# Jiawei-Yang/Denoising-ViT

Measured on AMD Instinct MI355X. Metric: stage-1 images denoised/sec (DINOv2-B/14, 518px, 1k Adam steps), higher is better.
Workload: dtype bf16

## Files before the change

### denoising-vit_amd/csrc/dvt_common.h

```cpp
#pragma once
#include <hip/hip_runtime.h>
#include <stdint.h>

#include "../../include/dvt_hip.h"

#define DVT_CHECK_LAUNCH()                         \
  do {                                             \
    hipError_t e__ = hipGetLastError();            \
    if (e__ != hipSuccess) return (int)e__;        \
  } while (0)

static inline int dvt_cdiv(long long a, long long b) { return (int)((a + b - 1) / b); }

__device__ __forceinline__ float wave_sum(float v) {
#pragma unroll
  for (int o = 32; o > 0; o >>= 1) v += __shfl_xor(v, o, 64);
  return v;
}

__device__ __forceinline__ double wave_sum_f64(double v) {
#pragma unroll
  for (int o = 32; o > 0; o >>= 1) v += __shfl_xor(v, o, 64);
  return v;
}
// ... 131 lines not shown
          t[dvt_frag_off32(k + 0, n, N)] = v.x;
          t[dvt_frag_off32(k + 1, n, N)] = v.y;
          t[dvt_frag_off32(k + 2, n, N)] = v.z;
          t[dvt_frag_off32(k + 3, n, N)] = v.w;
        }
        continue;
      }
      const uint32_t lo = dvt_pack_bf16x2(v.x, v.y), hi = dvt_pack_bf16x2(v.z, v.w);
      *reinterpret_cast<uint2*>(sh + L.direct[i] + dvt_frag_off(n, k, K)) = make_uint2(lo, hi);
      if (L.transp[i] >= 0) {
        uint16_t* t = sh + L.transp[i];
        t[dvt_frag_off(k + 0, n, N)] = (uint16_t)(lo & 0xffffu);
        t[dvt_frag_off(k + 1, n, N)] = (uint16_t)(lo >> 16);
        t[dvt_frag_off(k + 2, n, N)] = (uint16_t)(hi & 0xffffu);
        t[dvt_frag_off(k + 3, n, N)] = (uint16_t)(hi >> 16);
      }
    }
  }
}
#endif
bool dvt_fit_fused_ok(const DvtFitConfig* c);
bool dvt_fit_fused_shapes_ok(const DvtFitConfig* c);
int dvt_fit_rows_k(const DvtFitConfig* c, const DvtShadowLayout* L, int k, const DvtFusedFit* fits, bool phase2,
                   hipStream_t s);
int dvt_fit_backward_k(const DvtFitConfig* c, int k, const DvtFusedFit* fits, bool phase2, hipStream_t s);

extern unsigned g_dvt_prof_mask;
long dvt_prof_begin(int probe, hipStream_t s, unsigned long long* gen);
void dvt_prof_end(int probe, long idx, unsigned long long gen, hipStream_t s, double work);
struct DvtProbeScope {
  int probe;
  hipStream_t s;
  double work;
  long idx;
  unsigned long long gen;
  DvtProbeScope(int p, hipStream_t st, double w) : probe(p), s(st), work(w), idx(-1), gen(0) {
    if ((g_dvt_prof_mask >> p) & 1u) idx = dvt_prof_begin(probe, s, &gen);
  }
  ~DvtProbeScope() {
    if (idx >= 0) dvt_prof_end(probe, idx, gen, s, work);
  }
};
int dvt_vit_tune(int gemm_variant);
int dvt_grid_tune(int lds_level_max);
int dvt_adam_tune(int zero_all);
int dvt_s2_tune(int mask);

// ... 33 lines not shown
```

### denoising-vit_amd/csrc/dvt_fit.hip

```cpp
#include <math.h>

#include "dvt_common.h"
#include "dvt_grid_dev.h"

extern int g_fit_sorted_grid;
#ifdef DVT_LAB
int g_fit_skip_mask = 0;
#endif
int g_fit_lazy_adam = 1;
int g_fit_shadow_in_adam = 1;
int g_fit_lazy_merge = 1;
int g_fit_lazy_exact = 0;
int g_fit_lazy_refresh = 32;

int g_adam_pingpong = 1;

namespace {

inline int64_t up256(int64_t x) { return (x + 255) / 256 * 256; }

struct Work {
  float *enc, *h1, *F, *raw, *dF, *dh1, *denc, *rows, *r1, *r2, *Hres, *dH, *dr2, *dr1;
  int32_t* g_offs;
  uint16_t* g_perm;
  void* shadow;
  void* T;
  uint32_t* gs_keys;
  uint16_t* gs_pay;
// ... 157 lines not shown
  return dvt_linear_fwd(h1, params + c->off_w2, params + c->off_b2, out, n, c->feat_dim,
                        c->hidden, 0, s);
}

namespace {

#define DVT_TRY(x)         \
  do {                     \
    int rc__ = (x);        \
    if (rc__) return rc__; \
  } while (0)

int check_bufs(const DvtFitConfig* c, const DvtFitBuffers* b, int step_begin, int step_end) {
  int rc = check_cfg(c);
  if (rc) return rc;
  if (!b || !b->feat || !b->xy || !b->idx || !b->params || !b->adam_m || !b->adam_v ||
      !b->grads || !b->touched || !b->workspace || !b->h_lr)
    return DVT_E_BADARG;
  if (step_begin < 0 || step_end > c->num_iters || step_begin > step_end) return DVT_E_BADARG;
  return 0;
}

int fit_step(const DvtFitConfig* c, int k, const DvtFitBuffers* const* bs, const Work* ws, int step,
             int gs_local, uint32_t lazy_e0, const DvtAdamLazy* lazy_next, int lazy_target, bool fused, hipStream_t s) {
  const int B = c->batch, C = c->feat_dim, H = c->hidden, R = c->res_hidden;
  const int E = c->grid.n_levels * c->grid.n_features;
  const bool phase2 = step > c->switch_step;
  const bool use_res = phase2 && c->enable_residual;
  constexpr int KM = DVT_FIT_BATCH_MAX;
  const float* xy[KM];
  const int32_t* ridx[KM];
  const float* feat[KM];
  float *P[KM], *Gd[KM], *M[KM], *V[KM];
  uint32_t* touched[KM];
  for (int f = 0; f < k; ++f) {
    xy[f] = bs[f]->xy;
    ridx[f] = bs[f]->idx + (size_t)step * B;
    feat[f] = bs[f]->feat;
    P[f] = bs[f]->params;
    Gd[f] = bs[f]->grads;
    M[f] = bs[f]->adam_m;
    V[f] = bs[f]->adam_v;
    touched[f] = bs[f]->touched;
  }
  auto at = [&](float* const* base, int64_t off, float** out) {
    for (int f = 0; f < k; ++f) out[f] = base[f] + off;
  };
// ... 20 lines not shown
    return o;
  };
  DvtLinearOp ops[4 * KM];
  int n_ops;
  auto launch = [&]() { return dvt_linear_group(ops, n_ops, s, c->mlp_bf16); };
  DvtShadowLayout shl{};
  void* shadow[KM] = {nullptr, nullptr, nullptr, nullptr};
  DvtFusedFit ff[KM];
  if (fused) {
    DVT_TRY(dvt_shadow_layout(c, &shl));
    for (int f = 0; f < k; ++f) {
      const Work& w = ws[f];
      shadow[f] = w.shadow;
      const size_t gso = (size_t)gs_local * c->grid.n_levels * 4 * B;
      const bool gs = w.gs_keys != nullptr && gs_local >= 0;
      ff[f] = DvtFusedFit{xy[f], ridx[f], feat[f], P[f], w.shadow, w.T, w.F, w.Hres, w.dF, w.denc, w.rows, Gd[f],
                          w.g_offs + (size_t)step * (c->lattice + 1), w.g_perm + (size_t)step * B, touched[f],
                          gs ? w.gs_keys + gso : nullptr, gs ? w.gs_pay + gso : nullptr, gs ? w.gs_w + gso : nullptr,
                          lazy_e0};
    }
#ifdef DVT_LAB
    if (!(g_fit_skip_mask & 1))
#endif
    DVT_TRY(dvt_fit_rows_k(c, &shl, k, ff, use_res, s));
  } else {
  {
    float* gridp[KM];
    at(P, c->off_grid, gridp);
    DVT_TRY(dvt_fit_prep_k(&c->grid, k, xy, ridx, gridp, enc, feat, raw, B, C, s));
  }
  n_ops = 0;
  for (int f = 0; f < k; ++f) {
    const Work& w = ws[f];
    ops[n_ops++] = fwd_op(f, w.enc, c->off_w1, c->off_b1, w.h1, H, E, 1);
    if (use_res) ops[n_ops++] = fwd_op(f, w.raw, c->off_wh1, c->off_bh1, w.r1, R, C, 1);
  }
  DVT_TRY(launch());
  n_ops = 0;
  for (int f = 0; f < k; ++f) {
    const Work& w = ws[f];
    ops[n_ops++] = fwd_op(f, w.h1, c->off_w2, c->off_b2, w.F, C, H, 0);
    if (use_res) ops[n_ops++] = fwd_op(f, w.r1, c->off_wh2, c->off_bh2, w.r2, R, R, 1);
  }
  DVT_TRY(launch());
  if (use_res) {
    n_ops = 0;
    for (int f = 0; f < k; ++f) ops[n_ops++] = fwd_op(f, ws[f].r2, c->off_wh3, c->off_bh3, ws[f].Hres, C, R, 0);
// ... 144 lines not shown
  return dvt_fit_run_batched(c, 1, &b, step_begin, step_end, stream);
}

extern "C" int dvt_fit_run_batched(const DvtFitConfig* c, int k, const DvtFitBuffers* const* bufs,
                                   int step_begin, int step_end, void* stream) {
  if (k <= 0 || k > DVT_FIT_BATCH_MAX || !bufs) return DVT_E_BADARG;
  Work w[DVT_FIT_BATCH_MAX];
  for (int j = 0; j < k; ++j) {
    int rc = check_bufs(c, bufs[j], step_begin, step_end);
    if (rc) return rc;
    for (int i = 0; i < j; ++i)
      if (bufs[i]->params == bufs[j]->params || bufs[i]->workspace == bufs[j]->workspace)
        return DVT_E_BADARG;
    carve(c, bufs[j]->workspace, &w[j]);
    if (w[j].g_offs != nullptr && step_begin < c->switch_step + 1) {
      const int last = step_end < c->switch_step + 1 ? step_end : c->switch_step + 1;
      rc = dvt_build_row_lists(bufs[j]->idx + (size_t)step_begin * c->batch, last - step_begin, c->batch,
                               c->lattice, w[j].g_offs + (size_t)step_begin * (c->lattice + 1),
                               w[j].g_perm + (size_t)step_begin * c->batch, (hipStream_t)stream);
      if (rc) return rc;
    }
  }
  const bool fused = dvt_fit_fused_ok(c) && w[0].shadow != nullptr && w[0].g_offs != nullptr;
  if (fused && step_end > step_begin) {
    DvtShadowLayout L;
    int rc = dvt_shadow_layout(c, &L);
    if (rc) return rc;
    const float* pp[DVT_FIT_BATCH_MAX];
    void* ss[DVT_FIT_BATCH_MAX];
    for (int j = 0; j < k; ++j) {
      pp[j] = bufs[j]->params;
      ss[j] = w[j].shadow;
    }
    rc = dvt_shadow_build_k(&L, k, pp, ss, 0, c->arena_floats, (hipStream_t)stream);
    if (rc) return rc;
  }
  const bool sorted_lists = g_fit_fused_enable_lists(c) && w[0].g_offs != nullptr && w[0].gs_keys != nullptr && g_fit_sorted_grid;
  uint32_t lazy_e0 = 0xffffffffu;
  int lazy_l0 = 0;
  DvtAdamLazy lz{};
  const int n_call = step_end - step_begin;
  const bool lazy = sorted_lists && g_fit_lazy_adam && w[0].lazy_done != nullptr && n_call >= 1 && n_call <= 65535 &&
                    lazy_range(c, &lazy_e0, &lazy_l0);
  if (!lazy) lazy_e0 = 0xffffffffu;
  if (lazy) {
    lz.e0 = lazy_e0;
// ... 47 lines not shown
          uc[j] = w[j].gs_ucount;
        }
        int rc = dvt_grid_sort_k(&c->grid, k, xy, ridx, c->batch, steps, keys, pay, ww, (hipStream_t)stream,
                                 lazy ? uk : nullptr, lazy ? uc : nullptr);
        if (rc) return rc;
      }
    }
    if (lazy && step > step_begin && (step - step_begin) % g_fit_lazy_refresh == 0) {
      int rc = dvt_adam_lazy_k(&lz, k, true, step - step_begin, nullptr, nullptr, (hipStream_t)stream);
      if (rc) return rc;
    } else if (lazy && step > step_begin && !merged_catchup) {
      const uint32_t* uk[DVT_FIT_BATCH_MAX];
      const int32_t* uc[DVT_FIT_BATCH_MAX];
      for (int j = 0; j < k; ++j) {
        uk[j] = w[j].gs_ukeys + (size_t)gs_local * c->grid.n_levels * 4 * c->batch;
        uc[j] = w[j].gs_ucount + (size_t)gs_local * c->grid.n_levels;
      }
      int rc = dvt_adam_lazy_k(&lz, k, false, step - step_begin, uk, uc, (hipStream_t)stream);
      if (rc) return rc;
    }
    const int rel_next = step + 1 - step_begin;
    merged_catchup = lazy && g_fit_lazy_merge && step + 1 < step_end && gs_local + 1 < GS_CHUNK &&
                     rel_next % g_fit_lazy_refresh != 0;
    int rc = fit_step(c, k, bufs, w, step, gs_local, lazy_e0, merged_catchup ? &lz : nullptr, rel_next, fused, (hipStream_t)stream);
    if (rc) return rc;
  }
  if (lazy) {
    int rc = dvt_adam_lazy_k(&lz, k, true, n_call, nullptr, nullptr, (hipStream_t)stream);
    if (rc) return rc;
  }
  return 0;
}
```

### denoising-vit_amd/csrc/dvt_fit_fused.hip

```cpp
#include "dvt_common.h"
#include "dvt_grid_dev.h"
#include "dvt_loss_row.h"

typedef short bf16x8 __attribute__((ext_vector_type(8)));
typedef float f32x4 __attribute__((ext_vector_type(4)));

int g_fit_rows32 = 1;
int g_fit_xcd_affinity = 1;
int g_fit_small_wg = 0;

namespace {

constexpr int FR0 = 16;
constexpr int FW8 = 8;
constexpr int FE = 128;

template <bool F32>
struct Op {
  static constexpr int ES = F32 ? 4 : 2;
  static constexpr int KS = F32 ? 16 : 32;
};
typedef unsigned u32x4f __attribute__((ext_vector_type(4)));

template <bool F32>
__host__ __device__ constexpr int apitch(int K) { return K * Op<F32>::ES + 16; }

struct FusedArgs {
  DvtGridTable T;
  DvtShadowLayout S;
  DvtTLayout TL;
  int n, lattice;
// ... 16 lines not shown
      const int sg = brow >> 4, g = (brow >> 2) & 3;
      float4 v;
      v.x = *reinterpret_cast<const float*>(src);
      v.y = *reinterpret_cast<const float*>(src + apitch<F32>(NC));
      v.z = *reinterpret_cast<const float*>(src + 2 * apitch<F32>(NC));
      v.w = *reinterpret_cast<const float*>(src + 3 * apitch<F32>(NC));
      const long long off = ((long long)(col >> 4) * (B >> 4) + sg) * 256 + (((g << 4) + (col & 15)) << 2);
      *reinterpret_cast<float4*>(static_cast<float*>(dstTv) + off) = v;
    } else {
      const int kstep = brow >> 5, g = (brow >> 3) & 3;
      uint32_t w[4];
#pragma unroll
      for (int j = 0; j < 4; ++j) {
        const uint32_t lo = *reinterpret_cast<const uint16_t*>(src + (2 * j) * apitch<F32>(NC));
        const uint32_t hi = *reinterpret_cast<const uint16_t*>(src + (2 * j + 1) * apitch<F32>(NC));
        w[j] = lo | (hi << 16);
      }
      const long long off = ((long long)(col >> 4) * (B >> 5) + kstep) * 512 + (((g << 4) + (col & 15)) << 3);
      *reinterpret_cast<uint4*>(static_cast<uint16_t*>(dstTv) + off) = make_uint4(w[0], w[1], w[2], w[3]);
    }
  }
}

template <int K, int N, bool RELU, bool MASK, int RB, int FW, bool F32>
__device__ __forceinline__ void mlp_layer(const char* actA, const void* __restrict__ Wv,
                                          const float* __restrict__ bias, char* act_out,
                                          float* __restrict__ gout, const char* mask, int wave, int lane) {
  constexpr int KS = Op<F32>::KS, ES = Op<F32>::ES;
  constexpr int NTILES = N / 16, NT = (NTILES + FW - 1) / FW, S = K / KS;
  constexpr int INFL = FW == 8 ? 24 : 16;
  constexpr int PD0 = INFL / NT > 16 ? 16 : (INFL / NT < 1 ? 1 : INFL / NT);
  constexpr int PD = PD0 < S ? PD0 : S;
  static_assert(K % KS == 0 && N % 16 == 0, "layer shape");
  const int lc = lane & 15, g = lane >> 4;
  f32x4 acc[RB][NT];
  const char* wp[NT];
#pragma unroll
  for (int i = 0; i < NT; ++i) {
#pragma unroll
    for (int rb = 0; rb < RB; ++rb) acc[rb][i] = (f32x4){0.f, 0.f, 0.f, 0.f};
    const int t = wave + FW * i;
    const int tt = (NTILES % FW == 0 || t < NTILES) ? t : 0;
    wp[i] = static_cast<const char*>(Wv) + (size_t)tt * S * 1024 + lane * 16;
  }
  u32x4f b[PD][NT];
#pragma unroll
  for (int p = 0; p < PD; ++p)
#pragma unroll
    for (int i = 0; i < NT; ++i) b[p][i] = *reinterpret_cast<const u32x4f*>(wp[i] + 1024 * p);
  __builtin_amdgcn_sched_barrier(0);
  const char* ap = actA + lc * apitch<F32>(K) + g * 16;
#pragma unroll
  for (int s = 0; s < S; ++s) {
    u32x4f av[RB];
#pragma unroll
    for (int rb = 0; rb < RB; ++rb) av[rb] = *reinterpret_cast<const u32x4f*>(ap + rb * 16 * apitch<F32>(K) + s * 64);
    if constexpr (F32) {
#pragma unroll
      for (int j = 0; j < 4; ++j)
#pragma unroll
        for (int i = 0; i < NT; ++i)
#pragma unroll
          for (int rb = 0; rb < RB; ++rb)
            acc[rb][i] = __builtin_amdgcn_mfma_f32_16x16x4f32(__uint_as_float(av[rb][j]), __uint_as_float(b[s % PD][i][j]),
                                                              acc[rb][i], 0, 0, 0);
    } else {
#pragma unroll
      for (int i = 0; i < NT; ++i)
#pragma unroll
        for (int rb = 0; rb < RB; ++rb)
          acc[rb][i] = __builtin_amdgcn_mfma_f32_16x16x32_bf16(__builtin_bit_cast(bf16x8, av[rb]),
                                                               __builtin_bit_cast(bf16x8, b[s % PD][i]), acc[rb][i], 0, 0, 0);
    }
    if (s + PD < S) {
#pragma unroll
      for (int i = 0; i < NT; ++i) b[s % PD][i] = *reinterpret_cast<const u32x4f*>(wp[i] + 1024 * (s + PD));
    }
    __builtin_amdgcn_sched_barrier(0);
  }
#pragma unroll
  for (int i = 0; i < NT; ++i) {
    const int t = wave + FW * i;
    if (NTILES % FW != 0 && t >= NTILES) continue;
    const int n = t * 16 + lc;
    const float bv = bias != nullptr ? bias[n] : 0.f;
#pragma unroll
    for (int rb = 0; rb < RB; ++rb)
#pragma unroll
      for (int r = 0; r < 4; ++r) {
        const int row = rb * 16 + 4 * g + r;
        float v = acc[rb][i][r] + bv;
        if (RELU) v = fmaxf(v, 0.f);
        if (MASK) {
          if constexpr (F32) {
            v = *reinterpret_cast<const float*>(mask + row * apitch<F32>(N) + n * ES) > 0.f ? v : 0.f;
          } else {
            const uint16_t m = *reinterpret_cast<const uint16_t*>(mask + row * apitch<F32>(N) + n * ES);
            v = (m != 0 && !(m & 0x8000u)) ? v : 0.f;
          }
        }
        if (act_out != nullptr) {
          if constexpr (F32) *reinterpret_cast<float*>(act_out + row * apitch<F32>(N) + n * ES) = v;
          else *reinterpret_cast<uint16_t*>(act_out + row * apitch<F32>(N) + n * ES) = bf16_of(v);
        }
        if (gout != nullptr) gout[(size_t)row * N + n] = v;
      }
  }
}

template <int C, bool PH2, int FR, bool F32 = false>
struct FusedLds {
  static constexpr int H = C / 2, R = C / 4;
  static constexpr int O_ENC = 0;
  static constexpr int O_H1 = O_ENC + FR * apitch<F32>(FE);
  static constexpr int O_DF = O_H1 + FR * apitch<F32>(H);
  static constexpr int O_RAW = O_DF + FR * apitch<F32>(C);
  static constexpr int O_R1 = O_RAW + FR * apitch<F32>(C);
  static constexpr int O_R2 = O_R1 + FR * apitch<F32>(R);
  static constexpr int TOTAL = PH2 ? O_R2 + FR * apitch<F32>(R) : O_RAW;
};
template <int C>
constexpr bool fused_f32_fits() { return FusedLds<C, true, 16, true>::TOTAL <= 160 * 1024; }

template <int C, bool PH2, int FR, int FW, bool F32 = false>
__global__ __launch_bounds__(64 * FW) void fit_rows_kernel(FusedArgs a) {
  using L = FusedLds<C, PH2, FR, F32>;
  constexpr int RB = FR / 16;
  constexpr int ES = Op<F32>::ES;
  static_assert(FR == 16 || FR == 32, "rows per workgroup");
  static_assert(FW == 8 || (FW == 4 && FR == 16), "waves per workgroup");
  static_assert(!F32 || (FR == 16 && FW == 8), "fp32 operands: 16 rows, 8 waves");
  static_assert(L::TOTAL <= 160 * 1024, "LDS images of the row kernel");
  constexpr int H = C / 2, R = C / 4, E = FE, cq = C / 4;
  __shared__ __attribute__((aligned(16))) char smem[L::TOTAL];
  int fit_, rb_;
  if (a.xcd_group > 0) {
    const int lin = (int)blockIdx.x + (int)blockIdx.y * (int)gridDim.x, xcd = lin & 7, j = lin >> 3;
    fit_ = xcd / a.xcd_group;
    rb_ = j * a.xcd_group + xcd % a.xcd_group;
  } else {
    fit_ = (int)blockIdx.y;
    rb_ = (int)blockIdx.x;
  }
  const DvtFusedFit& f = a.f[fit_];
  const int tid = threadIdx.x, lane = tid & 63;
  const int wave = __builtin_amdgcn_readfirstlane(tid >> 6);
  const int row0 = rb_ * FR;
// ... 9 lines not shown
    for (int rr = lane / 32; rr < FR / FW; rr += 2) {
      if (j < LPR) {
        const int ri = f.ridx[row0 + wave + FW * rr];
        warm[4] ^= __float_as_uint(f.feat[(size_t)ri * C + j * 32]) ^
                   __float_as_uint(P[a.off_G + (size_t)(ri % a.lattice) * C + j * 32]);
      }
    }
  }
  {
    const int per_xcd = a.xcd_group > 0 ? (int)gridDim.x / a.xcd_group : ((int)gridDim.x + 7) / 8;
    const int nslot = per_xcd >= 16 ? 16 : per_xcd;
    const int slot = (a.xcd_group > 0 ? rb_ / a.xcd_group : (rb_ >> 3)) % nslot;
    const long long lines = ((PH2 ? a.S.total : a.S.direct[2]) * ES + 127) / 128;
    const long long per = (lines + nslot - 1) / nslot;
    const long long l0 = slot * per, l1 = l0 + per < lines ? l0 + per : lines;
    const uint32_t* w32 = reinterpret_cast<const uint32_t*>(sh);
#pragma unroll
    for (int j = 0; j < 4 * RB * (8 / FW); ++j) {
      const long long li = l0 + tid + (long long)j * 64 * FW;
      if (li < l1) warm[j & 3] ^= w32[li * 32];
    }
  }

  if (tid < FR * 16) {
    const int r = tid >> 4, l = tid & 15;
    const float2 p = reinterpret_cast<const float2*>(f.xy)[f.ridx[row0 + r]];
    uint32_t idx[4];
    float w[4];
    corners2d(a.T, l, p.x, p.y, idx, w);
    const float4* __restrict__ grid = reinterpret_cast<const float4*>(P + a.off_grid);
    float4 lo = make_float4(0.f, 0.f, 0.f, 0.f), hi = lo;
#pragma unroll
    for (int c = 0; c < 4; ++c) {
      const float4 u = grid[(size_t)idx[c] * 2], v = grid[(size_t)idx[c] * 2 + 1];
      lo.x = fmaf(w[c], u.x, lo.x);
      lo.y = fmaf(w[c], u.y, lo.y);
      lo.z = fmaf(w[c], u.z, lo.z);
      lo.w = fmaf(w[c], u.w, lo.w);
      hi.x = fmaf(w[c], v.x, hi.x);
      hi.y = fmaf(w[c], v.y, hi.y);
      hi.z = fmaf(w[c], v.z, hi.z);
      hi.w = fmaf(w[c], v.w, hi.w);
    }
    if constexpr (F32) {
      *reinterpret_cast<float4*>(smem + L::O_ENC + r * apitch<F32>(E) + l * 32) = lo;
      *reinterpret_cast<float4*>(smem + L::O_ENC + r * apitch<F32>(E) + l * 32 + 16) = hi;
    } else {
      *reinterpret_cast<uint4*>(smem + L::O_ENC + r * apitch<F32>(E) + l * 16) =
          make_uint4(dvt_pack_bf16x2(lo.x, lo.y), dvt_pack_bf16x2(lo.z, lo.w), dvt_pack_bf16x2(hi.x, hi.y),
                     dvt_pack_bf16x2(hi.z, hi.w));
    }
  }
  if (PH2) {
    for (int i = tid; i < FR * cq; i += 64 * FW) {
      const int r = i / cq, q = i - r * cq;
      const float4 v = feat4[(size_t)f.ridx[row0 + r] * cq + q];
      if constexpr (F32)
        *reinterpret_cast<float4*>(smem + L::O_RAW + r * apitch<F32>(C) + q * 16) = v;
      else
        *reinterpret_cast<uint2*>(smem + L::O_RAW + r * apitch<F32>(C) + q * 8) =
            make_uint2(dvt_pack_bf16x2(v.x, v.y), dvt_pack_bf16x2(v.z, v.w));
    }
  }
  __syncthreads();

  const int B = a.n;
  char* __restrict__ T = static_cast<char*>(f.T);
#define SH(off) (sh + (size_t)(off) * ES)
#define TT(idx) (T + (size_t)a.TL.off[idx] * ES)
  mlp_layer<E, H, true, false, RB, FW, F32>(smem + L::O_ENC, SH(a.S.direct[0]), P + a.off_b1, smem + L::O_H1, nullptr,
                               nullptr, wave, lane);
  if (PH2)
    mlp_layer<C, R, true, false, RB, FW, F32>(smem + L::O_RAW, SH(a.S.direct[2]), P + a.off_bh1, smem + L::O_R1, nullptr,
                                 nullptr, wave, lane);
  __syncthreads();
  mlp_layer<H, C, false, false, RB, FW, F32>(smem + L::O_H1, SH(a.S.direct[1]), P + a.off_b2, nullptr,
                                f.F + (size_t)row0 * C, nullptr, wave, lane);
  store_T<H, FR, FW, F32>(smem + L::O_H1, TT(DVT_T_H1), B, row0, tid);
  store_T<E, FR, FW, F32>(smem + L::O_ENC, TT(DVT_T_ENC), B, row0, tid);
  if (PH2) {
    mlp_layer<R, R, true, false, RB, FW, F32>(smem + L::O_R1, SH(a.S.direct[3]), P + a.off_bh2, smem + L::O_R2, nullptr,
                                 nullptr, wave, lane);
    store_T<C, FR, FW, F32>(smem + L::O_RAW, TT(DVT_T_RAW), B, row0, tid);
    store_T<R, FR, FW, F32>(smem + L::O_R1, TT(DVT_T_R1), B, row0, tid);
    __syncthreads();
    mlp_layer<R, C, false, false, RB, FW, F32>(smem + L::O_R2, SH(a.S.direct[4]), P + a.off_bh3, nullptr,
                                  f.Hres + (size_t)row0 * C, nullptr, wave, lane);
    store_T<R, FR, FW, F32>(smem + L::O_R2, TT(DVT_T_R2), B, row0, tid);
  }
  __syncthreads();

  static_assert(C <= 1024, "row warm-up above assumes <= 32 lines per row");
  {
    constexpr int NR = FR / FW;
    constexpr int NB = (C <= 768 && !(FW == 4 && PH2)) ? 2 : 1;
    DvtLossRowRegs<PH2> lr[NB];
#pragma unroll
    for (int r0 = 0; r0 < NR; r0 += NB) {
#pragma unroll
    for (int rr = r0; rr < r0 + NB; ++rr) {
      const int gr = row0 + wave + FW * rr;
      const int ri = f.ridx[gr];
      dvt_loss_row_load<PH2>(lr[rr - r0], reinterpret_cast<const float4*>(f.F) + (size_t)gr * cq,
                             reinterpret_cast<const float4*>(P + a.off_G) + (size_t)(ri % a.lattice) * cq,
                             PH2 ? reinterpret_cast<const float4*>(f.Hres) + (size_t)gr * cq : nullptr,
                             feat4 + (size_t)ri * cq, cq, lane);
    }
#pragma unroll
    for (int rr = r0; rr < r0 + NB; ++rr) {
      const int row = wave + FW * rr, gr = row0 + row;
      char* const img_p = smem + L::O_DF + row * apitch<F32>(C);
      char* const img_h = PH2 ? smem + L::O_RAW + row * apitch<F32>(C) : nullptr;
      dvt_loss_row_compute<PH2>(lr[rr - r0], reinterpret_cast<float4*>(f.dF) + (size_t)gr * cq,
                                nullptr, nullptr,
                                f.rows + (size_t)gr * 8, a.n, cq, a.grad_scale, lane,
                                F32 ? nullptr : reinterpret_cast<uint2*>(img_p), F32 ? nullptr : reinterpret_cast<uint2*>(img_h),
                                F32 ? reinterpret_cast<float4*>(img_p) : nullptr, F32 ? reinterpret_cast<float4*>(img_h) : nullptr);
    }
    }
  }
  __syncthreads();

  mlp_layer<C, H, false, true, RB, FW, F32>(smem + L::O_DF, SH(a.S.transp[1]), nullptr, smem + L::O_H1, nullptr,
                               smem + L::O_H1, wave, lane);
  store_T<C, FR, FW, F32>(smem + L::O_DF, TT(DVT_T_DF), B, row0, tid);
  if (PH2) {
    mlp_layer<C, R, false, true, RB, FW, F32>(smem + L::O_RAW, SH(a.S.transp[4]), nullptr, smem + L::O_R2, nullptr,
                                 smem + L::O_R2, wave, lane);
    store_T<C, FR, FW, F32>(smem + L::O_RAW, TT(DVT_T_DH), B, row0, tid);
  }
  __syncthreads();
  mlp_layer<H, E, false, false, RB, FW, F32>(smem + L::O_H1, SH(a.S.transp[0]), nullptr, nullptr,
                                f.denc + (size_t)row0 * E, nullptr, wave, lane);
  store_T<H, FR, FW, F32>(smem + L::O_H1, TT(DVT_T_DH1), B, row0, tid);
  if (PH2) {
    mlp_layer<R, R, false, true, RB, FW, F32>(smem + L::O_R2, SH(a.S.transp[3]), nullptr, smem + L::O_R1, nullptr,
                                 smem + L::O_R1, wave, lane);
    store_T<R, FR, FW, F32>(smem + L::O_R2, TT(DVT_T_DR2), B, row0, tid);
    __syncthreads();
    store_T<R, FR, FW, F32>(smem + L::O_R1, TT(DVT_T_DR1), B, row0, tid);
  }
#undef SH
#undef TT
  if (a.n < 0) f.rows[tid] = __uint_as_float(warm[0] ^ warm[1] ^ warm[2] ^ warm[3] ^ warm[4]);
}

__global__ __launch_bounds__(256) void shadow_build_kernel(DvtShadowLayout L, const float* const p0,
                                                           const float* const p1, const float* const p2,
                                                           const float* const p3, void* s0, void* s1,
                                                           void* s2, void* s3, long long q_lo, long long q_hi) {
  const float* p = blockIdx.y == 0 ? p0 : (blockIdx.y == 1 ? p1 : (blockIdx.y == 2 ? p2 : p3));
  void* sh = blockIdx.y == 0 ? s0 : (blockIdx.y == 1 ? s1 : (blockIdx.y == 2 ? s2 : s3));
  const long long q = q_lo + (long long)blockIdx.x * 256 + threadIdx.x;
  if (q >= q_hi) return;
  dvt_shadow_store(L, sh, q * 4, reinterpret_cast<const float4*>(p)[q]);
}


constexpr int WG_MAX_PROB = 5 * DVT_FIT_BATCH_MAX;
struct WgradProb {
// ... 175 lines not shown
  GridSortedPtrs gs;
  int n, grid_blocks_per_fit, k, wg_blocks;
  WgradArgs w;
};
template <int WAVES, bool F32 = false>
__global__ __launch_bounds__(64 * WAVES) void fit_backward_kernel(BackwardArgs a) {
  __shared__ __attribute__((aligned(16))) float smem[WAVES * WG_PART_FLOATS];
  if ((int)blockIdx.x >= a.wg_blocks) {
    const int b = (int)blockIdx.x - a.wg_blocks;
    const int fy = b / a.grid_blocks_per_fit, bx = b - fy * a.grid_blocks_per_fit;
    if (a.gs.nt > 0) {
      const int parts = a.gs.nt / (64 * WAVES);
      grid_gather_body(a.T, a.gs, fy, bx / parts, bx % parts, a.gp.d_enc[fy], a.gp.d_params[fy], a.gp.touched[fy], 64 * WAVES);
      return;
    }
    if constexpr (WAVES == 16)
      grid_bwd_body<256>(a.T, a.plan, a.gp, a.n, bx, fy, smem, reinterpret_cast<uint32_t*>(smem + 256 * 8));
    return;
  }
  const int wave = __builtin_amdgcn_readfirstlane(threadIdx.x >> 6);
  wgrad_block<WAVES / 4, F32>(a.w, (int)blockIdx.x, wave, threadIdx.x & 63, smem);
}

template <int C>
int launch_rows(const FusedArgs& a, int k, bool phase2, hipStream_t s) {
  if (a.S.f32) {
    if constexpr (fused_f32_fits<C>()) {
      dim3 grid(a.n / 16, k), block(64 * FW8);
      if (phase2) hipLaunchKernelGGL((fit_rows_kernel<C, true, 16, FW8, true>), grid, block, 0, s, a);
      else hipLaunchKernelGGL((fit_rows_kernel<C, false, 16, FW8, true>), grid, block, 0, s, a);
      DVT_CHECK_LAUNCH();
      return 0;
    }
    return DVT_E_BADARG;
  }
  const bool fits32 = phase2 ? (FusedLds<C, true, 32>::TOTAL <= 160 * 1024) : (FusedLds<C, false, 32>::TOTAL <= 160 * 1024);
  const bool r32 = fits32 && a.n % 32 == 0 && (g_fit_rows32 == 2 || (g_fit_rows32 == 1 && k >= 4));
  const bool small = g_fit_small_wg && !r32;
  dim3 grid(a.n / (r32 ? 32 : 16), k), block(64 * (small ? 4 : FW8));
  FusedArgs ax = a;
  ax.xcd_group = (g_fit_xcd_affinity && (k == 2 || k == 4) && grid.x % (8 / k) == 0 && (grid.x * k) % 8 == 0) ? 8 / k : 0;
  const FusedArgs& a_ = ax;
  if (r32) {
    if (phase2) {
      if constexpr (FusedLds<C, true, 32>::TOTAL <= 160 * 1024) hipLaunchKernelGGL((fit_rows_kernel<C, true, 32, FW8>), grid, block, 0, s, a_);
    } else {
      if constexpr (FusedLds<C, false, 32>::TOTAL <= 160 * 1024) hipLaunchKernelGGL((fit_rows_kernel<C, false, 32, FW8>), grid, block, 0, s, a_);
    }
  } else if (small) {
    if (phase2) hipLaunchKernelGGL((fit_rows_kernel<C, true, 16, 4>), grid, block, 0, s, a_);
    else hipLaunchKernelGGL((fit_rows_kernel<C, false, 16, 4>), grid, block, 0, s, a_);
  } else if (phase2) {
    hipLaunchKernelGGL((fit_rows_kernel<C, true, 16, FW8>), grid, block, 0, s, a_);
  } else {
    hipLaunchKernelGGL((fit_rows_kernel<C, false, 16, FW8>), grid, block, 0, s, a_);
  }
  DVT_CHECK_LAUNCH();
  return 0;
}

}

int dvt_shadow_layout(const DvtFitConfig* c, DvtShadowLayout* L) {
  if (!c || !L) return DVT_E_BADARG;
  const int C = c->feat_dim, H = c->hidden, R = c->res_hidden;
  const int E = c->grid.n_levels * c->grid.n_features;
  const int Ns[DVT_SHADOW_MATS] = {H, C, R, R, C}, Ks[DVT_SHADOW_MATS] = {E, H, C, R, R};
  const long long begins[DVT_SHADOW_MATS] = {c->off_w1, c->off_w2, c->off_wh1, c->off_wh2, c->off_wh3};
  const bool tr[DVT_SHADOW_MATS] = {true, true, false, true, true};
  long long o = 0;
  L->n = DVT_SHADOW_MATS;
  L->f32 = c->mlp_bf16 ? 0 : 1;
  L->lo = begins[0];
  L->hi = 0;
  for (int i = 0; i < DVT_SHADOW_MATS; ++i) {
    if (Ks[i] % 32 || Ns[i] % 16 || (tr[i] && (Ns[i] % 32 || Ks[i] % 16))) return DVT_E_BADARG;
    L->N[i] = Ns[i];
    L->K[i] = Ks[i];
// ... 30 lines not shown

int g_fit_fused_enable = 1;
int g_fit_sorted_grid = 1;

int g_fit_fused_f32 = 1;

bool dvt_fit_fused_ok(const DvtFitConfig* c) {
  if (!g_fit_fused_enable || !c || !dvt_fit_fused_shapes_ok(c)) return false;
  if (c->mlp_bf16) return true;
  return g_fit_fused_f32 && (c->feat_dim == 384 || c->feat_dim == 768);
}

bool dvt_fit_fused_shapes_ok(const DvtFitConfig* c) {
  if (!c) return false;
  if (c->grid.n_levels != 16 || c->grid.n_features != 8) return false;
  const int C = c->feat_dim;
  if (C != 384 && C != 768 && C != 1024) return false;
  if (c->hidden != C / 2 || c->res_hidden != C / 4) return false;
  if (c->batch % 512 || c->batch <= 0) return false;
  return c->lattice <= 8192 && c->batch <= 65535;
}

int dvt_fit_rows_k(const DvtFitConfig* c, const DvtShadowLayout* L, int k, const DvtFusedFit* fits, bool phase2,
                   hipStream_t s) {
  if (!dvt_fit_fused_ok(c) || !L || !fits || k < 1 || k > DVT_FIT_BATCH_MAX) return DVT_E_BADARG;
  FusedArgs a{};
  a.T = c->grid;
  a.S = *L;
  dvt_t_layout(c, &a.TL);
  a.n = c->batch;
  a.lattice = c->lattice;
  a.grad_scale = (float)c->grad_scale;
  a.off_grid = c->off_grid;
  a.off_b1 = c->off_b1;
  a.off_b2 = c->off_b2;
  a.off_G = c->off_G;
  a.off_bh1 = c->off_bh1;
  a.off_bh2 = c->off_bh2;
  a.off_bh3 = c->off_bh3;
  for (int f = 0; f < k; ++f) a.f[f] = fits[f];
  const double C = c->feat_dim, H = c->hidden, R = c->res_hidden, E = FE, B = c->batch;
  const double flops = 2.0 * B * (2.0 * (E * H + H * C) + (phase2 ? (C * R + 2.0 * R * R + 2.0 * R * C) : 0.0));
  DvtProbeScope probe(DVT_PROBE_FIT_ROWS, s, flops * k);
  switch (c->feat_dim) {
    case 384: return launch_rows<384>(a, k, phase2, s);
    case 768: return launch_rows<768>(a, k, phase2, s);
    default: return launch_rows<1024>(a, k, phase2, s);
  }
}

void dvt_t_layout(const DvtFitConfig* c, DvtTLayout* L) {
  const int C = c->feat_dim, H = c->hidden, R = c->res_hidden, E = c->grid.n_levels * c->grid.n_features;
  const int cols[DVT_T_COUNT] = {C, H, H, E, C, R, R, C, R, R};
  long long o = 0;
  for (int i = 0; i < DVT_T_COUNT; ++i) {
    L->off[i] = o;
    L->cols[i] = cols[i];
    o += (long long)cols[i] * c->batch;
  }
  L->total = o;
}

int dvt_fit_backward_k(const DvtFitConfig* c, int k, const DvtFusedFit* fits, bool phase2, hipStream_t s) {
  if (!dvt_fit_fused_ok(c) || !fits || k < 1 || k > DVT_FIT_BATCH_MAX) return DVT_E_BADARG;
  DvtTLayout TL;
  dvt_t_layout(c, &TL);
  const int C = c->feat_dim, H = c->hidden, R = c->res_hidden, E = c->grid.n_levels * c->grid.n_features;
  BackwardArgs ba{};
  WgradArgs& a = ba.w;
  a.B = c->batch;
// ... 82 lines not shown
```

### denoising-vit_amd/csrc/dvt_gemm_f32.hip

```cpp
#include "dvt_common.h"

typedef float floatx16 __attribute__((ext_vector_type(16)));

namespace {

constexpr int BK = 64;
constexpr int LDK = BK + 4;

struct GemmArgs {
  const float* A;
  const float* B;
  float* C;
  int M, N, K;
  int lda, ldb, ldc;
  const float* bias;
  const float* mask;
  int ldmask;
  float* colsum;
  int relu;
  int kchunk;
  int atomic;
  int epi;
  const float* gamma;
  const float* smul;
// ... 778 lines not shown
  else if (g_f32_bk == 32)
    hipLaunchKernelGGL(gemm_f32_multi_kernel<32>, dim3(blocks), dim3(256), 0, s, m);
  else
    hipLaunchKernelGGL(gemm_f32_multi_kernel<64>, dim3(blocks), dim3(256), 0, s, m);
  DVT_CHECK_LAUNCH();
  return 0;
}

namespace {
extern int g_cfg_override;
}
extern int g_fit_fused_enable;
extern int g_fit_fused_f32;
extern int g_fit_sorted_grid;
extern int g_fit_lazy_adam;
extern int g_fit_lazy_refresh;
extern int g_fit_lazy_exact;
extern int g_fit_lazy_merge;
extern int g_fit_shadow_in_adam;
extern int g_adam_pingpong;
extern int g_fit_rows32;
extern int g_fit_small_wg;
extern int g_fit_xcd_affinity;
#ifdef DVT_LAB
extern int g_fit_skip_mask;
#endif

extern "C" int dvt_tune_set(int key, int value) {
  if (key == 0) {
    g_cfg_override = value;
    return 0;
  }
  if (key == 4) {
    if (value == 2 || value == 3)
      g_f32_ex_stages = value;
    else if (value == 10 || value == 11)
      g_f32_big = value == 11;
    else
      g_f32_glds = value;
    return 0;
  }
  if (key == 5) {
    if (value != 16 && value != 32 && value != 64) return DVT_E_BADARG;
    g_f32_bk = value;
    return 0;
  }
// ... 15 lines not shown
  if (key == 10) {
    g_fit_lazy_exact = value != 0;
    return 0;
  }
  if (key == 11) {
    g_fit_lazy_merge = value != 0;
    return 0;
  }
  if (key == 12) {
    g_fit_shadow_in_adam = value != 0;
    return 0;
  }
  if (key == 13) {
    if (value < 0 || value > 2) return DVT_E_BADARG;
    g_fit_rows32 = value;
    return 0;
  }
  if (key == 14) {
    g_fit_small_wg = value != 0;
    return 0;
  }
  if (key == 16) {
    g_fit_xcd_affinity = value != 0;
    return 0;
  }
#ifdef DVT_LAB
  if (key == 15) {
    g_fit_skip_mask = value & 7;
    return 0;
  }
#endif
  if (key == 9) {
    g_fit_lazy_adam = value != 0;
    if (value >= 2) g_fit_lazy_refresh = value;
    return 0;
  }
  if (key == 18) return dvt_s2_tune(value);
  if (key == 1) return dvt_vit_tune(value);
  if (key == 2) return dvt_grid_tune(value);
  if (key == 3) return dvt_adam_tune(value);
  return DVT_E_BADARG;
}

int dvt_gemm_f32_ex(const DvtGemmEx* g, hipStream_t s) {
  if (!g || !g->A || !g->B || !g->C || g->M <= 0 || g->N <= 0 || g->K <= 0) return DVT_E_BADARG;
  GemmArgs a{};
// ... 180 lines not shown
```

Before: 2.938.

## Prefetch next layer's weight tiles during current layer's tail in fused fit kernel

Adds a chained mode to the fused fit-rows kernel. During the last pipeline steps of each MLP layer, the first weight fragments of the next layer are loaded into a register head buffer, and the kernel prologue preloads the first layer's weights before the input encoding. This hides the weight-load latency at layer boundaries. The change also hoists bias loads ahead of the MMA loop and skips the dF write in phase 2. The cost is higher register pressure from the 24-entry head buffer and extra template instantiations. A tune key toggles the mode, and it is on by default.

```diff
diff --git a/denoising-vit_amd/csrc/dvt_common.h b/denoising-vit_amd/csrc/dvt_common.h
--- a/denoising-vit_amd/csrc/dvt_common.h
+++ b/denoising-vit_amd/csrc/dvt_common.h
@@ -177,7 +177,7 @@
 bool dvt_fit_fused_ok(const DvtFitConfig* c);
 bool dvt_fit_fused_shapes_ok(const DvtFitConfig* c);
 int dvt_fit_rows_k(const DvtFitConfig* c, const DvtShadowLayout* L, int k, const DvtFusedFit* fits, bool phase2,
-                   hipStream_t s);
+                   bool chained, hipStream_t s);
 int dvt_fit_backward_k(const DvtFitConfig* c, int k, const DvtFusedFit* fits, bool phase2, hipStream_t s);
 
 extern unsigned g_dvt_prof_mask;
diff --git a/denoising-vit_amd/csrc/dvt_fit.hip b/denoising-vit_amd/csrc/dvt_fit.hip
--- a/denoising-vit_amd/csrc/dvt_fit.hip
+++ b/denoising-vit_amd/csrc/dvt_fit.hip
@@ -4,6 +4,7 @@
 #include "dvt_grid_dev.h"
 
 extern int g_fit_sorted_grid;
+extern int g_fit_stream;
 #ifdef DVT_LAB
 int g_fit_skip_mask = 0;
 #endif
@@ -207,7 +208,8 @@
 }
 
 int fit_step(const DvtFitConfig* c, int k, const DvtFitBuffers* const* bs, const Work* ws, int step,
-             int gs_local, uint32_t lazy_e0, const DvtAdamLazy* lazy_next, int lazy_target, bool fused, hipStream_t s) {
+             int gs_local, uint32_t lazy_e0, const DvtAdamLazy* lazy_next, int lazy_target, bool fused, bool chained,
+             hipStream_t s) {
   const int B = c->batch, C = c->feat_dim, H = c->hidden, R = c->res_hidden;
   const int E = c->grid.n_levels * c->grid.n_features;
   const bool phase2 = step > c->switch_step;
@@ -274,7 +276,7 @@
 #ifdef DVT_LAB
     if (!(g_fit_skip_mask & 1))
 #endif
-    DVT_TRY(dvt_fit_rows_k(c, &shl, k, ff, use_res, s));
+    DVT_TRY(dvt_fit_rows_k(c, &shl, k, ff, use_res, chained, s));
   } else {
   {
     float* gridp[KM];
@@ -465,6 +467,7 @@
     }
   }
   const bool fused = dvt_fit_fused_ok(c) && w[0].shadow != nullptr && w[0].g_offs != nullptr;
+  const bool chained = g_fit_stream != 0;
   if (fused && step_end > step_begin) {
     DvtShadowLayout L;
     int rc = dvt_shadow_layout(c, &L);
@@ -558,7 +561,7 @@
     const int rel_next = step + 1 - step_begin;
     merged_catchup = lazy && g_fit_lazy_merge && step + 1 < step_end && gs_local + 1 < GS_CHUNK &&
                      rel_next % g_fit_lazy_refresh != 0;
-    int rc = fit_step(c, k, bufs, w, step, gs_local, lazy_e0, merged_catchup ? &lz : nullptr, rel_next, fused, (hipStream_t)stream);
+    int rc = fit_step(c, k, bufs, w, step, gs_local, lazy_e0, merged_catchup ? &lz : nullptr, rel_next, fused, chained, (hipStream_t)stream);
     if (rc) return rc;
   }
   if (lazy) {
diff --git a/denoising-vit_amd/csrc/dvt_fit_fused.hip b/denoising-vit_amd/csrc/dvt_fit_fused.hip
--- a/denoising-vit_amd/csrc/dvt_fit_fused.hip
+++ b/denoising-vit_amd/csrc/dvt_fit_fused.hip
@@ -7,6 +7,7 @@
 
 int g_fit_rows32 = 1;
 int g_fit_xcd_affinity = 1;
+int g_fit_stream = 1;
 int g_fit_small_wg = 0;
 
 namespace {
@@ -69,16 +70,51 @@
   }
 }
 
-template <int K, int N, bool RELU, bool MASK, int RB, int FW, bool F32>
+template <int K, int N, int FW, bool F32>
+struct WPipe {
+  static constexpr int KS = Op<F32>::KS;
+  static constexpr int NTILES = N / 16, NT = (NTILES + FW - 1) / FW, S = K / KS;
+  static constexpr int INFL = FW == 8 ? 24 : 16;
+  static constexpr int PD0 = INFL / NT > 16 ? 16 : (INFL / NT < 1 ? 1 : INFL / NT);
+  static constexpr int PD = PD0 < S ? PD0 : S;
+  static_assert(K % KS == 0 && N % 16 == 0, "layer shape");
+  static constexpr int head_steps(int cap) { return cap < PD ? (cap < 0 ? 0 : cap) : PD; }
+};
+
+constexpr int HEAD_MAX = 24;
+struct WHead {
+  u32x4f b[HEAD_MAX];
+};
+
+template <int K, int N, int FW, bool F32>
+__device__ __forceinline__ const char* wtile(const void* __restrict__ Wv, int i, int wave, int lane) {
+  using WP = WPipe<K, N, FW, F32>;
+  const int t = wave + FW * i;
+  const int tt = (WP::NTILES % FW == 0 || t < WP::NTILES) ? t : 0;
+  return static_cast<const char*>(Wv) + (size_t)tt * WP::S * 1024 + lane * 16;
+}
+template <int K, int N, int FW, bool F32>
+__device__ __forceinline__ void head_issue(WHead& hd, const void* __restrict__ Wv, int wave, int lane, int q_lo, int q_hi) {
+  using WP = WPipe<K, N, FW, F32>;
+  static_assert(WP::PD * WP::NT <= HEAD_MAX, "head buffer");
+#pragma unroll
+  for (int q = 0; q < WP::PD * WP::NT; ++q)
+    if (q >= q_lo && q < q_hi)
+      hd.b[q] = *reinterpret_cast<const u32x4f*>(wtile<K, N, FW, F32>(Wv, q % WP::NT, wave, lane) + 1024 * (q / WP::NT));
+}
+
+template <int K, int N, bool RELU, bool MASK, int RB, int FW, bool F32, bool CH = false, int HCAP = 0, int NK = 0, int NN = 0,
+          int NCAP = 0>
 __device__ __forceinline__ void mlp_layer(const char* actA, const void* __restrict__ Wv,
                                           const float* __restrict__ bias, char* act_out,
-                                          float* __restrict__ gout, const char* mask, int wave, int lane) {
-  constexpr int KS = Op<F32>::KS, ES = Op<F32>::ES;
-  constexpr int NTILES = N / 16, NT = (NTILES + FW - 1) / FW, S = K / KS;
-  constexpr int INFL = FW == 8 ? 24 : 16;
-  constexpr int PD0 = INFL / NT > 16 ? 16 : (INFL / NT < 1 ? 1 : INFL / NT);
-  constexpr int PD = PD0 < S ? PD0 : S;
-  static_assert(K % KS == 0 && N % 16 == 0, "layer shape");
+                                          float* __restrict__ gout, const char* mask, int wave, int lane,
+                                          WHead* hd = nullptr, const void* __restrict__ Wn = nullptr) {
+  using WP = WPipe<K, N, FW, F32>;
+  using WPN = WPipe<NK != 0 ? NK : Op<F32>::KS, NN != 0 ? NN : 16, FW, F32>;
+  constexpr int ES = Op<F32>::ES;
+  constexpr int NTILES = WP::NTILES, NT = WP::NT, S = WP::S, PD = WP::PD;
+  constexpr int HP = CH ? WP::head_steps(HCAP) : 0;
+  constexpr int NQ = (CH && NK != 0) ? WPN::head_steps(NCAP) * WPN::NT : 0;
   const int lc = lane & 15, g = lane >> 4;
   f32x4 acc[RB][NT];
   const char* wp[NT];
@@ -86,15 +122,24 @@
   for (int i = 0; i < NT; ++i) {
 #pragma unroll
     for (int rb = 0; rb < RB; ++rb) acc[rb][i] = (f32x4){0.f, 0.f, 0.f, 0.f};
-    const int t = wave + FW * i;
-    const int tt = (NTILES % FW == 0 || t < NTILES) ? t : 0;
-    wp[i] = static_cast<const char*>(Wv) + (size_t)tt * S * 1024 + lane * 16;
+    wp[i] = wtile<K, N, FW, F32>(Wv, i, wave, lane);
   }
   u32x4f b[PD][NT];
 #pragma unroll
   for (int p = 0; p < PD; ++p)
 #pragma unroll
-    for (int i = 0; i < NT; ++i) b[p][i] = *reinterpret_cast<const u32x4f*>(wp[i] + 1024 * p);
+    for (int i = 0; i < NT; ++i) {
+      if (p < HP) b[p][i] = hd->b[p * NT + i];
+      else b[p][i] = *reinterpret_cast<const u32x4f*>(wp[i] + 1024 * p);
+    }
+  float bvv[NT];
+  if constexpr (CH) {
+#pragma unroll
+    for (int i = 0; i < NT; ++i) {
+      const int t = wave + FW * i;
+      bvv[i] = (bias != nullptr && (NTILES % FW == 0 || t < NTILES)) ? bias[t * 16 + lc] : 0.f;
+    }
+  }
   __builtin_amdgcn_sched_barrier(0);
   const char* ap = actA + lc * apitch<F32>(K) + g * 16;
 #pragma unroll
@@ -122,6 +167,9 @@
     if (s + PD < S) {
 #pragma unroll
       for (int i = 0; i < NT; ++i) b[s % PD][i] = *reinterpret_cast<const u32x4f*>(wp[i] + 1024 * (s + PD));
+    } else if constexpr (NQ > 0) {
+      const int j = s - (S - PD);
+      head_issue<NK, NN, FW, F32>(*hd, Wn, wave, lane, j * NQ / PD, (j + 1) * NQ / PD);
     }
     __builtin_amdgcn_sched_barrier(0);
   }
@@ -130,7 +178,9 @@
     const int t = wave + FW * i;
     if (NTILES % FW != 0 && t >= NTILES) continue;
     const int n = t * 16 + lc;
-    const float bv = bias != nullptr ? bias[n] : 0.f;
+    float bv;
+    if constexpr (CH) bv = bvv[i];
+    else bv = bias != nullptr ? bias[n] : 0.f;
 #pragma unroll
     for (int rb = 0; rb < RB; ++rb)
 #pragma unroll
@@ -169,7 +219,7 @@
 template <int C>
 constexpr bool fused_f32_fits() { return FusedLds<C, true, 16, true>::TOTAL <= 160 * 1024; }
 
-template <int C, bool PH2, int FR, int FW, bool F32 = false>
+template <int C, bool PH2, int FR, int FW, bool F32 = false, bool CH = true>
 __global__ __launch_bounds__(64 * FW) void fit_rows_kernel(FusedArgs a) {
   using L = FusedLds<C, PH2, FR, F32>;
   constexpr int RB = FR / 16;
@@ -225,6 +275,15 @@
     }
   }
 
+#define SH(off) (sh + (size_t)(off) * ES)
+  constexpr int FULL = 16;
+  constexpr int LCAP = (PH2 && FW == 8 && C >= 768) ? (C == 768 ? 3 : 2) : FULL;
+  WHead hd;
+  if constexpr (CH) {
+    head_issue<E, H, FW, F32>(hd, SH(a.S.direct[0]), wave, lane, 0, HEAD_MAX);
+    __builtin_amdgcn_sched_barrier(0);
+  }
+
   if (tid < FR * 16) {
     const int r = tid >> 4, l = tid & 15;
     const float2 p = reinterpret_cast<const float2*>(f.xy)[f.ridx[row0 + r]];
@@ -269,26 +328,30 @@
 
   const int B = a.n;
   char* __restrict__ T = static_cast<char*>(f.T);
-#define SH(off) (sh + (size_t)(off) * ES)
 #define TT(idx) (T + (size_t)a.TL.off[idx] * ES)
-  mlp_layer<E, H, true, false, RB, FW, F32>(smem + L::O_ENC, SH(a.S.direct[0]), P + a.off_b1, smem + L::O_H1, nullptr,
-                               nullptr, wave, lane);
+  mlp_layer<E, H, true, false, RB, FW, F32, CH, FULL, PH2 ? C : H, PH2 ? R : C, FULL>(
+      smem + L::O_ENC, SH(a.S.direct[0]), P + a.off_b1, smem + L::O_H1, nullptr, nullptr, wave, lane, &hd,
+      PH2 ? SH(a.S.direct[2]) : SH(a.S.direct[1]));
   if (PH2)
-    mlp_layer<C, R, true, false, RB, FW, F32>(smem + L::O_RAW, SH(a.S.direct[2]), P + a.off_bh1, smem + L::O_R1, nullptr,
-                                 nullptr, wave, lane);
+    mlp_layer<C, R, true, false, RB, FW, F32, CH, FULL, H, C, FULL>(smem + L::O_RAW, SH(a.S.direct[2]), P + a.off_bh1,
+                                                                    smem + L::O_R1, nullptr, nullptr, wave, lane, &hd,
+                                                                    SH(a.S.direct[1]));
   __syncthreads();
-  mlp_layer<H, C, false, false, RB, FW, F32>(smem + L::O_H1, SH(a.S.direct[1]), P + a.off_b2, nullptr,
-                                f.F + (size_t)row0 * C, nullptr, wave, lane);
+  mlp_layer<H, C, false, false, RB, FW, F32, CH, FULL, PH2 ? R : C, PH2 ? R : H, PH2 ? FULL : LCAP>(
+      smem + L::O_H1, SH(a.S.direct[1]), P + a.off_b2, nullptr, f.F + (size_t)row0 * C, nullptr, wave, lane, &hd,
+      PH2 ? SH(a.S.direct[3]) : SH(a.S.transp[1]));
   store_T<H, FR, FW, F32>(smem + L::O_H1, TT(DVT_T_H1), B, row0, tid);
   store_T<E, FR, FW, F32>(smem + L::O_ENC, TT(DVT_T_ENC), B, row0, tid);
   if (PH2) {
-    mlp_layer<R, R, true, false, RB, FW, F32>(smem + L::O_R1, SH(a.S.direct[3]), P + a.off_bh2, smem + L::O_R2, nullptr,
-                                 nullptr, wave, lane);
+    mlp_layer<R, R, true, false, RB, FW, F32, CH, FULL, R, C, FULL>(smem + L::O_R1, SH(a.S.direct[3]), P + a.off_bh2,
+                                                                    smem + L::O_R2, nullptr, nullptr, wave, lane, &hd,
+                                                                    SH(a.S.direct[4]));
     store_T<C, FR, FW, F32>(smem + L::O_RAW, TT(DVT_T_RAW), B, row0, tid);
     store_T<R, FR, FW, F32>(smem + L::O_R1, TT(DVT_T_R1), B, row0, tid);
     __syncthreads();
-    mlp_layer<R, C, false, false, RB, FW, F32>(smem + L::O_R2, SH(a.S.direct[4]), P + a.off_bh3, nullptr,
-                                  f.Hres + (size_t)row0 * C, nullptr, wave, lane);
+    mlp_layer<R, C, false, false, RB, FW, F32, CH, FULL, C, H, LCAP>(smem + L::O_R2, SH(a.S.direct[4]), P + a.off_bh3, nullptr,
+                                                                     f.Hres + (size_t)row0 * C, nullptr, wave, lane, &hd,
+                                                                     SH(a.S.transp[1]));
     store_T<R, FR, FW, F32>(smem + L::O_R2, TT(DVT_T_R2), B, row0, tid);
   }
   __syncthreads();
@@ -314,7 +377,7 @@
       const int row = wave + FW * rr, gr = row0 + row;
       char* const img_p = smem + L::O_DF + row * apitch<F32>(C);
       char* const img_h = PH2 ? smem + L::O_RAW + row * apitch<F32>(C) : nullptr;
-      dvt_loss_row_compute<PH2>(lr[rr - r0], reinterpret_cast<float4*>(f.dF) + (size_t)gr * cq,
+      dvt_loss_row_compute<PH2>(lr[rr - r0], PH2 ? nullptr : reinterpret_cast<float4*>(f.dF) + (size_t)gr * cq,
                                 nullptr, nullptr,
                                 f.rows + (size_t)gr * 8, a.n, cq, a.grad_scale, lane,
                                 F32 ? nullptr : reinterpret_cast<uint2*>(img_p), F32 ? nullptr : reinterpret_cast<uint2*>(img_h),
@@ -324,21 +387,24 @@
   }
   __syncthreads();
 
-  mlp_layer<C, H, false, true, RB, FW, F32>(smem + L::O_DF, SH(a.S.transp[1]), nullptr, smem + L::O_H1, nullptr,
-                               smem + L::O_H1, wave, lane);
+  mlp_layer<C, H, false, true, RB, FW, F32, CH, LCAP, PH2 ? C : H, PH2 ? R : E, FULL>(
+      smem + L::O_DF, SH(a.S.transp[1]), nullptr, smem + L::O_H1, nullptr, smem + L::O_H1, wave, lane, &hd,
+      PH2 ? SH(a.S.transp[4]) : SH(a.S.transp[0]));
   store_T<C, FR, FW, F32>(smem + L::O_DF, TT(DVT_T_DF), B, row0, tid);
   if (PH2) {
-    mlp_layer<C, R, false, true, RB, FW, F32>(smem + L::O_RAW, SH(a.S.transp[4]), nullptr, smem + L::O_R2, nullptr,
-                                 smem + L::O_R2, wave, lane);
+    mlp_layer<C, R, false, true, RB, FW, F32, CH, FULL, H, E, FULL>(smem + L::O_RAW, SH(a.S.transp[4]), nullptr, smem + L::O_R2,
+                                                                    nullptr, smem + L::O_R2, wave, lane, &hd,
+                                                                    SH(a.S.transp[0]));
     store_T<C, FR, FW, F32>(smem + L::O_RAW, TT(DVT_T_DH), B, row0, tid);
   }
   __syncthreads();
-  mlp_layer<H, E, false, false, RB, FW, F32>(smem + L::O_H1, SH(a.S.transp[0]), nullptr, nullptr,
-                                f.denc + (size_t)row0 * E, nullptr, wave, lane);
+  mlp_layer<H, E, false, false, RB, FW, F32, CH, FULL, PH2 ? R : 0, PH2 ? R : 0, FULL>(
+      smem + L::O_H1, SH(a.S.transp[0]), nullptr, nullptr, f.denc + (size_t)row0 * E, nullptr, wave, lane, &hd,
+      PH2 ? SH(a.S.transp[3]) : nullptr);
   store_T<H, FR, FW, F32>(smem + L::O_H1, TT(DVT_T_DH1), B, row0, tid);
   if (PH2) {
-    mlp_layer<R, R, false, true, RB, FW, F32>(smem + L::O_R2, SH(a.S.transp[3]), nullptr, smem + L::O_R1, nullptr,
-                                 smem + L::O_R1, wave, lane);
+    mlp_layer<R, R, false, true, RB, FW, F32, CH, FULL>(smem + L::O_R2, SH(a.S.transp[3]), nullptr, smem + L::O_R1, nullptr,
+                                                        smem + L::O_R1, wave, lane, &hd);
     store_T<R, FR, FW, F32>(smem + L::O_R2, TT(DVT_T_DR2), B, row0, tid);
     __syncthreads();
     store_T<R, FR, FW, F32>(smem + L::O_R1, TT(DVT_T_DR1), B, row0, tid);
@@ -560,13 +626,13 @@
   wgrad_block<WAVES / 4, F32>(a.w, (int)blockIdx.x, wave, threadIdx.x & 63, smem);
 }
 
-template <int C>
+template <int C, bool CH>
 int launch_rows(const FusedArgs& a, int k, bool phase2, hipStream_t s) {
   if (a.S.f32) {
     if constexpr (fused_f32_fits<C>()) {
       dim3 grid(a.n / 16, k), block(64 * FW8);
-      if (phase2) hipLaunchKernelGGL((fit_rows_kernel<C, true, 16, FW8, true>), grid, block, 0, s, a);
-      else hipLaunchKernelGGL((fit_rows_kernel<C, false, 16, FW8, true>), grid, block, 0, s, a);
+      if (phase2) hipLaunchKernelGGL((fit_rows_kernel<C, true, 16, FW8, true, CH>), grid, block, 0, s, a);
+      else hipLaunchKernelGGL((fit_rows_kernel<C, false, 16, FW8, true, CH>), grid, block, 0, s, a);
       DVT_CHECK_LAUNCH();
       return 0;
     }
@@ -581,17 +647,17 @@
   const FusedArgs& a_ = ax;
   if (r32) {
     if (phase2) {
-      if constexpr (FusedLds<C, true, 32>::TOTAL <= 160 * 1024) hipLaunchKernelGGL((fit_rows_kernel<C, true, 32, FW8>), grid, block, 0, s, a_);
+      if constexpr (FusedLds<C, true, 32>::TOTAL <= 160 * 1024) hipLaunchKernelGGL((fit_rows_kernel<C, true, 32, FW8, false, CH>), grid, block, 0, s, a_);
     } else {
-      if constexpr (FusedLds<C, false, 32>::TOTAL <= 160 * 1024) hipLaunchKernelGGL((fit_rows_kernel<C, false, 32, FW8>), grid, block, 0, s, a_);
+      if constexpr (FusedLds<C, false, 32>::TOTAL <= 160 * 1024) hipLaunchKernelGGL((fit_rows_kernel<C, false, 32, FW8, false, CH>), grid, block, 0, s, a_);
     }
   } else if (small) {
-    if (phase2) hipLaunchKernelGGL((fit_rows_kernel<C, true, 16, 4>), grid, block, 0, s, a_);
-    else hipLaunchKernelGGL((fit_rows_kernel<C, false, 16, 4>), grid, block, 0, s, a_);
+    if (phase2) hipLaunchKernelGGL((fit_rows_kernel<C, true, 16, 4, false, CH>), grid, block, 0, s, a_);
+    else hipLaunchKernelGGL((fit_rows_kernel<C, false, 16, 4, false, CH>), grid, block, 0, s, a_);
   } else if (phase2) {
-    hipLaunchKernelGGL((fit_rows_kernel<C, true, 16, FW8>), grid, block, 0, s, a_);
+    hipLaunchKernelGGL((fit_rows_kernel<C, true, 16, FW8, false, CH>), grid, block, 0, s, a_);
   } else {
-    hipLaunchKernelGGL((fit_rows_kernel<C, false, 16, FW8>), grid, block, 0, s, a_);
+    hipLaunchKernelGGL((fit_rows_kernel<C, false, 16, FW8, false, CH>), grid, block, 0, s, a_);
   }
   DVT_CHECK_LAUNCH();
   return 0;
@@ -668,7 +734,7 @@
 }
 
 int dvt_fit_rows_k(const DvtFitConfig* c, const DvtShadowLayout* L, int k, const DvtFusedFit* fits, bool phase2,
-                   hipStream_t s) {
+                   bool chained, hipStream_t s) {
   if (!dvt_fit_fused_ok(c) || !L || !fits || k < 1 || k > DVT_FIT_BATCH_MAX) return DVT_E_BADARG;
   FusedArgs a{};
   a.T = c->grid;
@@ -689,9 +755,9 @@
   const double flops = 2.0 * B * (2.0 * (E * H + H * C) + (phase2 ? (C * R + 2.0 * R * R + 2.0 * R * C) : 0.0));
   DvtProbeScope probe(DVT_PROBE_FIT_ROWS, s, flops * k);
   switch (c->feat_dim) {
-    case 384: return launch_rows<384>(a, k, phase2, s);
-    case 768: return launch_rows<768>(a, k, phase2, s);
-    default: return launch_rows<1024>(a, k, phase2, s);
+    case 384: return chained ? launch_rows<384, true>(a, k, phase2, s) : launch_rows<384, false>(a, k, phase2, s);
+    case 768: return chained ? launch_rows<768, true>(a, k, phase2, s) : launch_rows<768, false>(a, k, phase2, s);
+    default: return chained ? launch_rows<1024, true>(a, k, phase2, s) : launch_rows<1024, false>(a, k, phase2, s);
   }
 }
 
diff --git a/denoising-vit_amd/csrc/dvt_gemm_f32.hip b/denoising-vit_amd/csrc/dvt_gemm_f32.hip
--- a/denoising-vit_amd/csrc/dvt_gemm_f32.hip
+++ b/denoising-vit_amd/csrc/dvt_gemm_f32.hip
@@ -824,6 +824,7 @@
 extern int g_fit_rows32;
 extern int g_fit_small_wg;
 extern int g_fit_xcd_affinity;
+extern int g_fit_stream;
 #ifdef DVT_LAB
 extern int g_fit_skip_mask;
 #endif
@@ -885,6 +886,10 @@
   }
   if (key == 16) {
     g_fit_xcd_affinity = value != 0;
+    return 0;
+  }
+  if (key == 17) {
+    g_fit_stream = value != 0;
     return 0;
   }
 #ifdef DVT_LAB
```

New measurement: 2.970 (median of 6 runs). +1.1%, better.
